# Srecharan/Leaf-Grasping-Vision-ML

Measured on AMD Instinct MI355X. Metric: frames/sec (1080p depth+mask) grasp scoring, 1/8 MI355X; % HBM roofline, higher is better.
Workload: dtype f32; 1 GPU; 1080x1920 depth+mask, 8 score planes + valid + top-20 NMS + GraspPointCNN fp32 rescoring of 20 candidates; height=1080, width=1920, batches_in_flight=1, parallelism=frames sharded over 1 GPU(s), no collective

## Files before the change

### include/leafgrasp.h

```cpp
#ifndef LEAFGRASP_H
#define LEAFGRASP_H

#include <stdint.h>

#ifdef __cplusplus
extern "C" {
#endif

typedef struct lg_ctx* lg_handle;

typedef enum lg_status {
    LG_OK = 0,
    LG_ERR_INVALID = -1,
    LG_ERR_HIP = -2,
    LG_ERR_NOMEM = -3,
    LG_ERR_NO_MODEL = -4,
    LG_ERR_UNSUPPORTED = -5,
    LG_ERR_BUSY = -6
} lg_status;

enum {
    LG_MAP_SDF = 0,
    LG_MAP_APPROACH = 1,
    LG_MAP_FLATNESS = 2,
// ... 161 lines not shown

int lg_debug_dt_max(lg_handle h, int frame, uint32_t out[2], int32_t win[4]);
int lg_debug_dt_form(lg_handle h, int frame, int32_t form[2]);
int lg_debug_dt_search_form(lg_handle h, int32_t* algo);
int lg_dt_form_host(int forced, int n, int H, int W);
int lg_debug_orient_redo(lg_handle h, int32_t* n);
int lg_near_tile_rect(int bx0, int bx1, int by0, int by1, int H, int W, int halo, int32_t rect[4]);
int lg_stem_words_host(const uint64_t* bits, int H, int W, int WW, int bottom_start, int k, uint64_t* out);
int lg_stem_words_host_spans(const uint64_t* bits, int H, int W, int WW, int bottom_start, int n, int anchor, const int8_t* lo,
                             const int8_t* hi, int algo, uint64_t* out);
int lg_stem_plan(int k, int n, int anchor, const int8_t* lo, const int8_t* hi, int32_t* i0, int8_t span_lo[64], int8_t span_hi[64],
                 int8_t dlo[64], int8_t dhi[64]);
int lg_window_from_box(const uint32_t box[5], int H, int W, int search_mode, int32_t out[12]);
int lg_border_line_max(const int32_t* prof, int n, int lo, int len, uint32_t* out);
int lg_debug_near_tiles(lg_handle h, int32_t* off, int cap);
int lg_debug_cnn_scored(lg_handle h, int64_t* patches);
int lg_debug_leaf_fallback(lg_handle h, int32_t* flags, int cap, int32_t* n_frames, int32_t* n_flagged);
int lg_debug_cnn_survivors(lg_handle h, int32_t* sub_frames, int32_t* n_sub, int32_t* counts, int32_t counts_cap,
                           int32_t* list, int32_t* slot, float* logits, int64_t cap, int64_t* n_slots);
int lg_debug_patch(lg_handle h, int64_t slot, float* out);
int lg_debug_isolation_fields(lg_handle h, int frame, uint32_t* dc_fix, uint32_t* dw_fix, uint32_t max_fix[2]);
int lg_label_aware_check(const lg_params* p, int has_labels);
int lg_norm3_host(const int32_t* dx, const int32_t* dy, int n, uint32_t* out);
int lg_dilate_words_host(const uint64_t* bits, int H, int W, int WW, int k, uint64_t* out);
int lg_debug_ws_plane_bytes(lg_handle h, int64_t bytes[LG_NUM_MAPS]);
int lg_wave_rows_on_mask(const uint64_t* bits, int H, int WW, int y, int w);

typedef struct lg_trainer lg_trainer;
typedef struct lg_train_hparams {
    float lr, beta1, beta2, eps, weight_decay;
// ... 40 lines not shown
```

### leaf-grasping-vision-ml_amd/_lib.py

```python
import ctypes as C
import os

_HERE = os.path.dirname(os.path.abspath(__file__))
LIB_PATH = os.environ.get("LG_LIB_PATH") or os.path.join(_HERE, "liblgrasp.so")

LG_NUM_MAPS = 8
MAP_NAMES = ("sdf_score", "approach_score", "flatness_map", "isolation_map", "distance_map",
             "accessibility_map", "stem_penalty", "traditional_score")
MAP_INDEX = {n: i for i, n in enumerate(MAP_NAMES)}

LG_OK, LG_ERR_INVALID, LG_ERR_HIP, LG_ERR_NOMEM, LG_ERR_NO_MODEL, LG_ERR_UNSUPPORTED, LG_ERR_BUSY = 0, -1, -2, -3, -4, -5, -6


class LgParams(C.Structure):
    _fields_ = [(n, C.c_double) for n in ("cx", "cy", "f")] + [(n, C.c_float) for n in (
        "w_approach", "w_sdf", "w_flat", "w_access", "sdf_w_interior", "sdf_w_align",
        "sdf_w_sdf", "optimal_distance", "access_w_dist", "access_w_dir", "flat_scale", "iso_w_close",
        "iso_w_wide", "iso_ramp_top", "iso_ramp_bottom", "min_edge_distance", "stem_valid_thresh")] + \
        [(n, C.c_int32) for n in ("stem_se", "stem_bottom_div", "top_k", "nms_min_distance",
                                  "pregrasp_clearance", "mask_is_bool", "gaussian_size", "chamfer_init_dist0", "label_aware")]


_FP = C.POINTER(C.c_float)

# ... 87 lines not shown
    "lg_debug_dt_max": (C.c_int, [_VP, C.c_int, C.POINTER(C.c_uint32), C.POINTER(C.c_int32)]),
    "lg_format_grasp_results": (C.c_int, [_VP, C.c_int, C.c_char_p, C.c_int64, C.POINTER(C.c_int64)]),
    "lg_debug_dt_form": (C.c_int, [_VP, C.c_int, C.POINTER(C.c_int32)]),
    "lg_debug_orient_redo": (C.c_int, [_VP, C.POINTER(C.c_int32)]),
    "lg_debug_dt_search_form": (C.c_int, [_VP, C.POINTER(C.c_int32)]),
    "lg_dt_form_host": (C.c_int, [C.c_int, C.c_int, C.c_int, C.c_int]),
    "lg_near_tile_rect": (C.c_int, [C.c_int, C.c_int, C.c_int, C.c_int, C.c_int, C.c_int, C.c_int, C.POINTER(C.c_int32)]),
    "lg_stem_words_host": (C.c_int, [_VP, C.c_int, C.c_int, C.c_int, C.c_int, C.c_int, _VP]),
    "lg_stem_words_host_spans": (C.c_int, [_VP, C.c_int, C.c_int, C.c_int, C.c_int, C.c_int, C.c_int, C.POINTER(C.c_int8),
                                           C.POINTER(C.c_int8), C.c_int, _VP]),
    "lg_stem_plan": (C.c_int, [C.c_int, C.c_int, C.c_int, C.POINTER(C.c_int8), C.POINTER(C.c_int8), C.POINTER(C.c_int32),
                               C.POINTER(C.c_int8), C.POINTER(C.c_int8), C.POINTER(C.c_int8), C.POINTER(C.c_int8)]),
    "lg_window_from_box": (C.c_int, [C.POINTER(C.c_uint32), C.c_int, C.c_int, C.c_int, C.POINTER(C.c_int32)]),
    "lg_border_line_max": (C.c_int, [C.POINTER(C.c_int32), C.c_int, C.c_int, C.c_int, C.POINTER(C.c_uint32)]),
    "lg_debug_near_tiles":(C.c_int, [_VP, C.POINTER(C.c_int32), C.c_int]),
    "lg_debug_cnn_scored": (C.c_int, [_VP, C.POINTER(C.c_int64)]),
    "lg_debug_leaf_fallback": (C.c_int, [_VP, C.POINTER(C.c_int32), C.c_int, C.POINTER(C.c_int32), C.POINTER(C.c_int32)]),
    "lg_debug_cnn_survivors": (C.c_int, [_VP, C.POINTER(C.c_int32), C.POINTER(C.c_int32), C.POINTER(C.c_int32), C.c_int32,
                                         C.POINTER(C.c_int32), C.POINTER(C.c_int32), _FP, C.c_int64, C.POINTER(C.c_int64)]),
    "lg_debug_patch": (C.c_int, [_VP, C.c_int64, _FP]),
    "lg_debug_isolation_fields": (C.c_int, [_VP, C.c_int, _VP, _VP, C.POINTER(C.c_uint32)]),
    "lg_label_aware_check": (C.c_int, [C.POINTER(LgParams), C.c_int]),
    "lg_norm3_host": (C.c_int, [_VP, _VP, C.c_int, _VP]),
    "lg_dilate_words_host": (C.c_int, [_VP, C.c_int, C.c_int, C.c_int, C.c_int, _VP]),
    "lg_debug_ws_plane_bytes": (C.c_int, [_VP, C.POINTER(C.c_int64)]),
    "lg_wave_rows_on_mask": (C.c_int, [_VP, C.c_int, C.c_int, C.c_int, C.c_int]),
    "lg_harvest_patches": (C.c_int, [_VP, _VP, _VP, _VP, C.c_int, C.c_int, C.c_int, _VP, _VP, _VP, _VP, _VP, _VP, _VP]),
    "lg_negative_masks": (C.c_int, [_VP, _VP, _VP, C.c_int, C.c_int, _VP, _VP, _VP]),
    "lg_leaf_contour": (C.c_int, [_VP, _VP, C.c_int, C.c_int, _VP, C.c_int, C.POINTER(C.c_int), _VP]),
    "lg_train_create": (C.c_int, [C.c_int, C.c_int, C.POINTER(C.c_int32), C.c_int, C.c_int, C.POINTER(_VP)]),
# ... 55 lines not shown
```

### leaf-grasping-vision-ml_amd/csrc/lg_api.hip

```cpp
#include <math.h>
#include <stdio.h>
#include <stdlib.h>
#include <string.h>

#include <algorithm>
#include <chrono>
#include <functional>
#include <string>
#include <atomic>
#include <memory>
#include <sched.h>
#include <condition_variable>
#include <mutex>
#include <thread>
#include <vector>

#include "lg_cnn.h"
#include "lg_dt.h"
#include "lg_eval.h"
#include "lg_leaf.h"
#include "lg_internal.h"
#include "lg_midrib.h"
#include "lg_orient.h"
#include "lg_pool.h"
// ... 20 lines not shown
    hipEvent_t ev_prep = nullptr, ev_copy = nullptr;
    hipStream_t s_dt[2] = {nullptr, nullptr}, s_main = nullptr, s_topk = nullptr;
    std::vector<hipEvent_t> ev_pool;
    hipEvent_t ev_begin = nullptr;
    int capB = 0, capH = 0, capW = 0, capK = 0;
    uint32_t* tmp = nullptr;
    unsigned long long *bits = nullptr, *stem = nullptr, *tilekeys = nullptr;
    uint8_t* tile_state = nullptr;
    int32_t* near_off = nullptr;
    int32_t* near_off_host = nullptr;
    hipEvent_t ev_near = nullptr;
    int32_t* near_off_host_dev = nullptr;
    LgFrameParams* fp_host_dev = nullptr;
    lg_grasp_result* res_host_dev = nullptr;
    int last_redo = 0;
    int last_near_B = 0;
    uint32_t* maxfix = nullptr;
    uint8_t* mask_ws = nullptr;
    size_t mask_ws_cap = 0;
    unsigned long long *iso_others = nullptr, *iso_dil = nullptr;
    uint32_t* iso_mf = nullptr;
    size_t iso_words_cap = 0;
    int iso_B_cap = 0;
    int last_iso_B = 0, last_iso_H = 0, last_iso_W = 0;
    int32_t* ids_dev = nullptr;
    int32_t* ids_host = nullptr;
    int ids_cap = 0;
    LgWin* win = nullptr;
    LgFrameParams* fp_dev = nullptr;
    LgFrameParams* fp_host = nullptr;
// ... 25 lines not shown
    LgOrientWs* orient = nullptr;
    hipEvent_t ev_orient = nullptr, ev_side = nullptr, ev_search = nullptr;
    int opt_dt_algo = 0;
    int last_dt_algo = 0;
    int opt_dt_band_p = 16, opt_dt_band_e = 4;
    int opt_dt_search = 2;
    int prof_on = 0;
    std::vector<LgProfSlot> prof;
    int host_threads = 8;
    LgPool* pool = nullptr;
    int opt_subbatch = 0;
    bool opt_trace = false;
    int opt_no_skip = 0;
    int opt_final_near = LG_FINAL_NEAR_TPW;
    bool opt_defer_planes = true;
    long long last_patch_floats = 0;
    bool opt_nt_stores = false;
    int opt_side_tail = 1;
    int opt_stem_algo = 1;
    bool opt_direct_host = true;
    bool export_pending = false;
    std::string orient_note;
    std::atomic<bool> busy{false};
    hipStream_t s_cnn = nullptr;
    hipEvent_t ev_cnn0 = nullptr, ev_cnn1 = nullptr;
    bool opt_host_orient = false;
    LgMidribWs* midrib = nullptr;
    void* eval_ws = nullptr;
    size_t eval_cap = 0;
};
// ... 72 lines not shown
        p.used = 0;
    }
}

template <typename T>
hipError_t dev_alloc(T** p, size_t n) {
    return hipMalloc((void**)p, n * sizeof(T));
}

void free_ws(lg_ctx* h) {
    auto F = [](void* p) { if (p) hipFree(p); };
    F(h->tmp); F(h->bits); F(h->stem); F(h->tilekeys); F(h->tile_state); F(h->maxfix); F(h->win); F(h->fp_dev);
    for (int i = 0; i < LG_NUM_MAPS; i++) { F(h->ws_maps_base[i]); h->ws_maps_base[i] = h->ws_maps[i] = nullptr; }
    F(h->ws_valid); F(h->cand_xy); F(h->cand_n); F(h->cand_info); F(h->patches); F(h->logits);
    F(h->surv_keep); F(h->surv_list); F(h->surv_slot); F(h->surv_count);
    F(h->near_off); h->near_off = nullptr; h->last_near_B = 0; h->last_iso_B = 0;
    h->surv_keep = nullptr; h->surv_list = h->surv_slot = h->surv_count = nullptr;
    h->last_scored = 0; h->last_scored_subs = 0; h->last_cnn_B = 0; h->last_patch_floats = 0;
    auto HF = [](void* p) { if (p) hipHostFree(p); };
    HF(h->fp_host); HF(h->bits_host); HF(h->win_host); HF(h->res_host); HF(h->near_off_host);
    h->near_off_host = nullptr;
    h->near_off_host_dev = nullptr; h->fp_host_dev = nullptr; h->res_host_dev = nullptr;
    F(h->res_dev);
    h->tmp = nullptr; h->bits = h->stem = h->tilekeys = nullptr; h->tile_state = nullptr; h->maxfix = nullptr; h->win = nullptr; h->fp_dev = nullptr;
    h->ws_valid = nullptr; h->cand_xy = h->cand_n = nullptr; h->cand_info = h->patches = h->logits = nullptr;
    h->fp_host = nullptr; h->bits_host = nullptr; h->win_host = nullptr; h->bits_host_dev = nullptr; h->res_dev = h->res_host = nullptr;
    h->capB = h->capH = h->capW = h->capK = 0;
}

int ensure_ws(lg_ctx* h, int B, int H, int W, int K) {
    if (B <= h->capB && H == h->capH && W == h->capW && K <= h->capK) return LG_OK;
// ... 141 lines not shown
        return LG_ERR_HIP;
    }
    unsigned hw = std::thread::hardware_concurrency();
    {
        cpu_set_t set;
        CPU_ZERO(&set);
        if (sched_getaffinity(0, sizeof(set), &set) == 0 && CPU_COUNT(&set) > 0) hw = (unsigned)CPU_COUNT(&set);
    }
    unsigned ranks = 1;
    if (const char* e = getenv("LOCAL_WORLD_SIZE")) ranks = (unsigned)std::max(1, atoi(e));
    h->host_threads = (int)std::max(1u, std::min((hw ? hw : 1u) / ranks, 16u));
    if (const char* e = getenv("LG_HOST_THREADS")) h->host_threads = std::max(1, atoi(e));
    if (const char* e = getenv("LG_SUBBATCH")) h->opt_subbatch = std::max(1, atoi(e));
    h->opt_trace = getenv("LG_TRACE") != nullptr;
    if (const char* e = getenv("LG_NO_SKIP")) h->opt_no_skip = std::max(1, atoi(e)) & 3;
    if (const char* e = getenv("LG_FINAL_NEAR")) h->opt_final_near = std::max(0, std::min(64, atoi(e)));
    if (getenv("LG_FINAL_PERSIST") || getenv("LG_FINAL_TPW")) h->opt_final_near = 0;
    h->opt_nt_stores = getenv("LG_NT_STORES") != nullptr;
    h->opt_host_orient = getenv("LG_HOST_ORIENT") != nullptr;
    if (const char* e = getenv("LG_CNN_PRUNE")) h->opt_cnn_prune = atoi(e) != 0;
    if (const char* e = getenv("LG_DEFER_PLANES")) h->opt_defer_planes = atoi(e) != 0;
    if (const char* e = getenv("LG_DT_SEARCH")) h->opt_dt_search = std::max(0, std::min(2, atoi(e)));
    if (const char* e = getenv("LG_DT_SEARCH_ALGO")) {
        const int f = atoi(e);
        if (f == 0 || f == LG_DT_FORM_ROWS || f == LG_DT_FORM_BANDS || f == LG_DT_FORM_SWEEP) h->opt_dt_algo = f;
    }
    if (const char* e = getenv("LG_DT_BAND_P")) { const int p = atoi(e); if (p == 12 || p == 16 || p == 24 || p == 32) h->opt_dt_band_p = p; }
    if (const char* e = getenv("LG_DT_BAND_E")) { const int v = atoi(e); if (v == 2 || v == 4) h->opt_dt_band_e = v; }
    if (const char* e = getenv("LG_SIDE_TAIL")) h->opt_side_tail = std::max(0, std::min(2, atoi(e)));
    if (const char* e = getenv("LG_STEM_ALGO")) h->opt_stem_algo = atoi(e) != 0;
// ... 318 lines not shown
    for (int i = 0; i < n; i++)
        if (prof[i] < -1 || prof[i] > 16384) return LG_ERR_INVALID;
    lg_border_search(prof, n, lo, len, out);
    return LG_OK;
}

int lg_debug_near_tiles(lg_handle h, int32_t* off, int cap) {
    if (!h || !off) return LG_ERR_INVALID;
    LG_ENTER(h);
    if (h->last_near_B <= 0 || !h->near_off_host) return fail(h, LG_ERR_INVALID, "lg_debug_near_tiles: the last call did not take the near launch");
    if (cap < h->last_near_B + 1) return fail(h, LG_ERR_INVALID, "lg_debug_near_tiles: cap must hold B + 1 entries");
    memcpy(off, h->near_off_host, sizeof(int32_t) * (h->last_near_B + 1));
    return LG_OK;
}

int lg_debug_orient_redo(lg_handle h, int32_t* n) {
    if (!h || !n) return LG_ERR_INVALID;
    LG_ENTER(h);
    *n = h->last_redo;
    return LG_OK;
}

int lg_debug_dt_form(lg_handle h, int frame, int32_t form[2]) {
    if (!h || !form || frame < 0 || frame >= h->capB || !h->win) return LG_ERR_INVALID;
    LG_ENTER(h);
    hipSetDevice(h->device);
    hipDeviceSynchronize();
    LgWin w;
    if (hipMemcpy(&w, h->win + frame, sizeof(w), hipMemcpyDeviceToHost) != hipSuccess)
        return fail(h, LG_ERR_HIP, "lg_debug_dt_form: copy failed");
// ... 92 lines not shown
    {
        LgSeSpans se;
        lg_make_se_spans(pl.P.stem_se, &se);
        const int third = pl.H / pl.P.stem_bottom_div;
        LgStemPlan sp;
        lg_make_stem_plan(se, &sp);
        ProfScope ps(h, "stem", s);
        lg_launch_stem_bits(h->bits + off * words, h->stem + off * words, h->win + off, n, pl.H, pl.W, pl.WW,
                            third ? pl.H - third : 0, se, h->opt_stem_algo ? &sp : nullptr, s);
    }
    return LG_OK;
}

int enq_prep(lg_ctx* h, const Plan& pl, int off, int n, hipStream_t s, hipEvent_t ev_prep) {
    h->export_pending = true;
    const size_t px = (size_t)pl.H * pl.W, words = (size_t)pl.H * pl.WW;
    LG_HIP(h, hipMemsetAsync(h->maxfix + LG_MF * (size_t)off, 0, sizeof(uint32_t) * LG_MF * n, s));
    if (pl.label_aware) LG_HIP(h, hipMemsetAsync(h->iso_mf + LG_ISO_MF * (size_t)off, 0, sizeof(uint32_t) * LG_ISO_MF * n, s));
    {
        ProfScope ps(h, "prep", s);
        if (pl.labels && pl.label_aware)
            lg_launch_pack_labels(pl.labels + off * px, h->ids_dev + off, h->mask_ws + off * px, h->bits + off * words, n, pl.H, pl.W,
                                  pl.WW, s, h->maxfix + LG_MF * (size_t)off, h->iso_others + off * words, h->iso_mf + LG_ISO_MF * (size_t)off);
        else if (pl.labels)
            lg_launch_pack_labels(pl.labels + off * px, h->ids_dev + off, h->mask_ws + off * px, h->bits + off * words, n, pl.H, pl.W,
                                  pl.WW, s, h->maxfix + LG_MF * (size_t)off);
        else
            lg_launch_pack_bits(pl.mask + off * px, h->bits + off * words, n, pl.H, pl.W, pl.WW, s, h->maxfix + LG_MF * (size_t)off);
    }
    {
// ... 161 lines not shown
    a.iso_w_close = P.iso_w_close; a.iso_w_wide = P.iso_w_wide;
    a.iso_ramp_top = P.iso_ramp_top; a.iso_ramp_bottom = P.iso_ramp_bottom;
    {
        uint32_t dmax = (uint32_t)((std::min(H, W) + 1) / 2);
        float mx = (float)((uint32_t)P.chamfer_init_dist0 + dmax * LG_A3) * (1.0f / 65536.0f);
        a.init0 = (uint32_t)P.chamfer_init_dist0;
        a.iso_inv_max = 1.0f / mx;
    }
    a.min_edge_distance = P.min_edge_distance; a.stem_valid_thresh = P.stem_valid_thresh;
    a.inv_maxd = (float)(1.0 / sqrt((double)W * W + (double)H * H));
    a.inv_2s2 = 1.0f / (2.0f * P.optimal_distance * P.optimal_distance);
    a.iso_ramp_step = (H > 1) ? (P.iso_ramp_bottom - P.iso_ramp_top) / (float)(H - 1) : 0.0f;
    gaussian1d(P.gaussian_size, a.k1);
    a.gauss_r = P.gaussian_size / 2;
    a.no_skip = h->opt_no_skip;
    a.persist = 0;
    a.nt_stores = h->opt_nt_stores ? 1 : 0;
    if (pl.near) {
        LG_HIP(h, hipEventSynchronize(h->ev_near));
        a.near_off = h->near_off;
        a.near_total = h->near_off_host[n];
        a.near_tpw = h->opt_final_near;
    }
    {
        ProfScope ps(h, "final", s, true);
        lg_launch_final(a, s, ps.slot ? ps.e0 : nullptr, ps.slot ? ps.e1 : nullptr);
    }
    if (keep) *keep = a;
    return LG_OK;
}
// ... 169 lines not shown
    for (int i = 0; i < n && i < cap; i++) { out_xy[2 * i] = pts[2 * i]; out_xy[2 * i + 1] = pts[2 * i + 1]; }
    return LG_OK;
}

int lg_leaf_orientation(lg_handle h, const uint8_t* mask, int H, int W, float* out, int* found, void* stream_) {
    if (!h) return LG_ERR_INVALID;
    LG_ENTER(h);
    if (!mask || !out || !found || H < 1 || W < 1) return fail(h, LG_ERR_INVALID, "lg_leaf_orientation: bad argument");
    hipStream_t s = (hipStream_t)stream_;
    LG_HIP(h, hipSetDevice(h->device));
    int rc = ensure_ws(h, 1, H, W, 20);
    if (rc) return rc;
    const int WW = (W + 63) / 64;
    LG_HIP(h, hipMemsetAsync(h->maxfix, 0, sizeof(uint32_t) * LG_MF, s));
    lg_launch_pack_bits(mask, h->bits, 1, H, W, WW, s, h->maxfix);
    double o[5];
    if (h->orient) {
        lg_launch_window(h->maxfix, h->win, 1, H, W, 0, s);
        lg_launch_orient(h->orient, h->bits, h->win, h->fp_dev, 0, 1, H, W, WW, s);
        LG_HIP(h, hipMemcpyAsync(h->orient->h_out, h->orient->out, sizeof(double) * 5, hipMemcpyDeviceToHost, s));
        LG_HIP(h, hipMemcpyAsync(h->orient->h_status, h->orient->status, sizeof(int), hipMemcpyDeviceToHost, s));
        LG_HIP(h, hipStreamSynchronize(s));
        if (!h->orient->h_status[0]) {
            *found = !std::isnan(h->orient->h_out[0]);
            for (int i = 0; i < 5; i++) out[i] = *found ? (float)h->orient->h_out[i] : NAN;
            return LG_OK;
        }
    }
    LG_HIP(h, hipMemcpyAsync(h->bits_host, h->bits, sizeof(unsigned long long) * (size_t)H * WW, hipMemcpyDeviceToHost, s));
    LG_HIP(h, hipStreamSynchronize(s));
// ... 463 lines not shown
            if (rc) return rc;
            pl.maps[i] = h->ws_maps[i];
        }
    if (!pl.valid) pl.valid = h->ws_valid;
    const int K = P.top_k;
    const size_t px = (size_t)H * W;
    const int tiles = pl.tiles_x * pl.tiles_y;

    int SB = B;
    if (h->opt_subbatch > 0 && !pl.label_aware) SB = h->opt_subbatch;
    const int nsub = (B + SB - 1) / SB;
    const bool piped = nsub > 1;
    std::vector<LgFinalArgs> fargs((size_t)nsub);
    pl.near = pl.sparse && h->opt_final_near > 0 && h->opt_subbatch == 0 && h->opt_no_skip == 0;
    h->last_near_B = 0;
    hipStream_t sD[2] = {piped ? h->s_dt[0] : s, piped ? h->s_dt[1] : s};
    hipStream_t sM = piped ? h->s_main : s, sT = piped ? h->s_topk : s;
    while ((int)h->ev_pool.size() < 6 * nsub) {
        hipEvent_t e;
        LG_HIP(h, hipEventCreateWithFlags(&e, hipEventDisableTiming));
        h->ev_pool.push_back(e);
    }
    auto EV = [&](int k, int which) { return h->ev_pool[6 * k + which]; };
    if (piped) {
        LG_HIP(h, hipEventRecord(h->ev_begin, s));
        for (hipStream_t q : {sD[0], sD[1], sM, sT}) LG_HIP(h, hipStreamWaitEvent(q, h->ev_begin, 0));
    }
    const LgIsoFields iso_fields = {h->tmp, h->iso_mf};
    auto enq_G = [&](int k) -> int {
        const int off = k * SB, n = std::min(SB, B - off);
// ... 129 lines not shown
    }
    if (!h->res_host_dev)
        LG_HIP(h, hipMemcpyAsync(h->res_host, h->res_dev, sizeof(lg_grasp_result) * B, hipMemcpyDeviceToHost, s));
    if (cands)
        LG_HIP(h, hipMemcpyAsync(h->cand_rows_host, h->cand_rows_dev, sizeof(lg_grasp_candidate) * B * K, hipMemcpyDeviceToHost, s));
    const double t_enq2 = now();
    LG_HIP(h, hipStreamSynchronize(s));
    const double t_sync = now();
    LG_HIP(h, hipGetLastError());
    if (use_cnn && lg_cnn_take_error(&h->cnn)) return fail(h, LG_ERR_HIP, "lg_select_grasp: a split CNN item did not receive its parts");
    memcpy(results, h->res_host, sizeof(lg_grasp_result) * B);
    if (cands) memcpy(cands, h->cand_rows_host, sizeof(lg_grasp_candidate) * B * K);
    if (use_cnn) { h->last_cnn_B = B; h->last_cnn_K = K; h->last_cnn_SB = SB; h->last_cnn_pruned = prune; }
    h->last_patch_floats = use_cnn ? (long long)B * K * lg_cnn_halo_patch_floats() : 0;
    if (pl.near) h->last_near_B = B;
    if (pl.label_aware) { h->last_iso_B = B; h->last_iso_H = H; h->last_iso_W = W; }
    if (trace && !piped) {
        float a[5] = {0};
        for (int i = 1; i <= 4; i++) hipEventElapsedTime(&a[i], tev[0], tev[i]);
        fprintf(stderr, "[lg] gpu timeline (ms since call start): sweeps done %.3f | planes %.3f | topk %.3f | cnn %.3f\n", a[1], a[2],
                a[3], a[4]);
    }
    if (trace) for (auto& e : tev) if (e) hipEventDestroy(e);
    if (trace)
        fprintf(stderr, "[lg] B=%d enq1 %.3f | wait bits %.3f | orient %.3f | enq2 %.3f | gpu wait %.3f | post %.3f ms\n", B,
                t_enq1 - t_start, t_copy - t_enq1, t_orient - t_copy, t_enq2 - t_orient, t_sync - t_enq2, now() - t_sync);
    return LG_OK;
}

}
// ... 1 lines not shown
```

### leaf-grasping-vision-ml_amd/csrc/lg_internal.h

```cpp
#pragma once
#include <hip/hip_runtime.h>
#include <stdint.h>

#include "../../include/leafgrasp.h"

#define LG_A5 65536u
#define LG_B5 91750u
#define LG_C5 143976u
#define LG_A3 62587u
#define LG_B3 89738u
#define LG_INIT0 0x1FFFFFFFu
#define LG_INF 0x3FFFFFFFu
#define LG_NOSRC 0x20000000u
#define LG_HCAP 16383u
#ifndef LG_SEARCH_BUDGET
#define LG_SEARCH_BUDGET 2.0e7f
#endif
#define LG_MF 8
#define LG_BOX_X0 2
#define LG_BOX_X1 3
#define LG_BOX_Y0 4
#define LG_BOX_Y1 5
#define LG_BOX_AREA 6

// ... 291 lines not shown
    float access_w_dist, access_w_dir, flat_scale;
    float iso_w_close, iso_w_wide, iso_ramp_top, iso_ramp_bottom, iso_inv_max;
    float min_edge_distance, stem_valid_thresh;
    float inv_maxd;
    uint32_t init0;
    float inv_2s2, iso_ramp_step;
    float k1[7];
    int gauss_r;
    int no_skip;
    int nt_stores;
    int persist;
    int tpw;
    const int32_t* near_off;
    int near_total;
    int near_tpw;
};

void lg_launch_pack_bits(const uint8_t* mask, unsigned long long* bits, int B, int H, int W, int WW, hipStream_t s,
                         uint32_t* mf = nullptr);
void lg_launch_pack_labels(const int16_t* labels, const int32_t* ids_dev, uint8_t* mask, unsigned long long* bits, int B, int H,
                           int W, int WW, hipStream_t s, uint32_t* mf = nullptr, unsigned long long* others = nullptr,
                           uint32_t* iso_mf = nullptr);
void lg_launch_export_rows(const unsigned long long* bits, const LgWin* wins, unsigned long long* dst_host_devptr, int B,
                           int H, int WW, hipStream_t s);
void lg_launch_stem_bits(const unsigned long long* bits, unsigned long long* stem, const LgWin* wins, int B, int H, int W, int WW,
                         int bottom_start, const LgSeSpans& se, const LgStemPlan* plan, hipStream_t s);
void lg_launch_final(const LgFinalArgs& a, hipStream_t s, hipEvent_t ev_start = nullptr, hipEvent_t ev_stop = nullptr);
void lg_launch_near_tiles(const LgWin* win, int B, int H, int W, int halo, int32_t* near_off, int32_t* near_off_host_dev,
                          unsigned long long* tilekeys, uint8_t* tile_state, hipStream_t s);
void lg_launch_smooth(const float* src, float* dst, int B, int H, int W, int S, const LgGaussTaps& taps, hipStream_t s);
// ... 99 lines not shown
```

### leaf-grasping-vision-ml_amd/csrc/lg_kernels.hip

```cpp
#include "lg_internal.h"
#include "lg_wave.h"

#include <hip/hip_ext.h>

#include <limits.h>
#include <algorithm>
#include <type_traits>
#include <stdlib.h>

#define LG_MAX64_STEP(CTRL, RMASK)                                                            \
    {                                                                                         \
        const uint32_t oh = (uint32_t)__builtin_amdgcn_update_dpp(0, (int)hi, CTRL, RMASK, 0xf, false); \
        const uint32_t ol = (uint32_t)__builtin_amdgcn_update_dpp(0, (int)lo, CTRL, RMASK, 0xf, false); \
        const bool take = (oh > hi) || (oh == hi && ol > lo);                                 \
        hi = take ? oh : hi;                                                                  \
        lo = take ? ol : lo;                                                                  \
    }
__device__ __forceinline__ unsigned long long lg_wave_max_u64(unsigned long long v) {
    uint32_t hi = (uint32_t)(v >> 32), lo = (uint32_t)v;
    LG_MAX64_STEP(0x111, 0xf)
    LG_MAX64_STEP(0x112, 0xf)
    LG_MAX64_STEP(0x114, 0xf)
    LG_MAX64_STEP(0x118, 0xf)
    LG_MAX64_STEP(0x142, 0xa)
// ... 89 lines not shown
        if (lane == 0) { fb[wid] = b; if (mf) acc.add(b, w * 64, row, H, W); }
    }
    if (mf) lg_box_flush(acc, s_box, mf + (size_t)frame * LG_MF);
}

__global__ __launch_bounds__(256) void lg_pack_bits16_kernel(const uint8_t* __restrict__ mask,
                                                             unsigned long long* __restrict__ bits, int H, int W, int WW,
                                                             uint32_t* __restrict__ mf) {
    __shared__ uint32_t s_box[5];
    const int slots_per_row = 4 * WW, frame = blockIdx.y;
    const int nslots = H * slots_per_row;
    const uint8_t* fm = mask + (size_t)frame * H * W;
    unsigned long long* fb = bits + (size_t)frame * H * WW;
    LgBoxAcc acc;
    const int stride = gridDim.x * 256;
    for (int sid = blockIdx.x * 256 + threadIdx.x; sid < nslots; sid += stride) {
        const int row = sid / slots_per_row;
        const int slot = sid - row * slots_per_row;
        const int x = slot * 16;
        unsigned b16 = 0;
        if (x < W) {
            const uint4 v = *reinterpret_cast<const uint4*>(fm + (size_t)row * W + x);
            const uint32_t w4[4] = {v.x, v.y, v.z, v.w};
#pragma unroll
            for (int q = 0; q < 4; q++) {
                b16 |= ((w4[q] & 0x000000ffu) ? 1u : 0u) << (4 * q);
                b16 |= ((w4[q] & 0x0000ff00u) ? 2u : 0u) << (4 * q);
                b16 |= ((w4[q] & 0x00ff0000u) ? 4u : 0u) << (4 * q);
                b16 |= ((w4[q] & 0xff000000u) ? 8u : 0u) << (4 * q);
            }
        }
        if (mf) acc.add(b16, x, row, H, W);
        unsigned long long word = (unsigned long long)b16 << (16 * (slot & 3));
        word |= __shfl_xor(word, 1, 64);
        word |= __shfl_xor(word, 2, 64);
        if ((slot & 3) == 0) fb[(size_t)row * WW + (slot >> 2)] = word;
    }
    if (mf) lg_box_flush(acc, s_box, mf + (size_t)frame * LG_MF);
}

static unsigned lg_pack_blocks(long long units, int B, long long target) {
    const long long full = (units + 255) / 256;
    return (unsigned)std::max<long long>(1, std::min<long long>(full, target / B));
}

void lg_launch_pack_bits(const uint8_t* mask, unsigned long long* bits, int B, int H, int W, int WW, hipStream_t s, uint32_t* mf) {
    if ((W & 15) == 0 && ((uintptr_t)mask & 15) == 0) {
        hipLaunchKernelGGL(lg_pack_bits16_kernel, dim3(lg_pack_blocks((long long)H * WW * 4, B, 16384), B), dim3(256), 0, s, mask, bits,
                           H, W, WW, mf);
        return;
    }
// ... 255 lines not shown

template <bool VEC, bool ALL, int R, bool SCORE = false>
__global__ __launch_bounds__(256) LG_FINAL_WPE_ATTR void lg_final_kernel(LgFinalArgs a_) {
    static_assert(!(ALL && SCORE), "score-only stores fewer planes than ALL");
    constexpr int HALO = R + 1;
    static_assert(R >= 0 && HALO <= 4, "the depth tile carries 4 halo columns");
    constexpr int DW = 72;
    constexpr int DH = LG_TH + 2 * HALO;
    constexpr int GW = LG_TW + 2;
    constexpr int GH = LG_TH + 2;
    __shared__ __attribute__((aligned(16))) float s_dm[DH * DW];
    __shared__ float s_h[DH * GW];
    float* const s_g = s_dm;
    static_assert(GH * (GW + 2) <= DH * DW, "g tile must fit in the depth tile");
    __shared__ unsigned long long s_key[4];
    __shared__ int s_any[2];
    typedef float lg_f4 __attribute__((ext_vector_type(4)));
    typedef const __attribute__((address_space(4))) LgFinalArgs* lg_args_ptr;
    lg_args_ptr ap = (lg_args_ptr)__builtin_amdgcn_kernarg_segment_ptr();
    (void)a_;

    const int ntile = ap->tiles_x * ap->tiles_y;
    typedef const __attribute__((address_space(4))) int32_t* lg_off_ptr;
    const bool near = ap->near_off != nullptr;
    const int total = near ? ap->near_total : ntile * ap->B;
    const int xcd = (int)(blockIdx.x & 7u), tq = total >> 3, tr = total & 7;
    const int xcd_first = xcd < tr ? xcd * (tq + 1) : tr * (tq + 1) + (xcd - tr) * tq;
    const int xcd_count = tq + (xcd < tr ? 1 : 0);
    const int tpw = near ? ap->near_tpw : ap->tpw;
    const int stride = tpw > 0 ? 1 : (int)((gridDim.x + 7u) >> 3);
    int it = (int)(blockIdx.x >> 3) * (tpw > 0 ? tpw : 1);
// ... 74 lines not shown
        }
    };
    auto st_valid = [&](unsigned off, int x0, uint32_t vbytes) {
        if (!ALL && !SCORE && !ap->valid) return;
        uint8_t* p = ap->valid + fo + off;
        if (vec) {
            __builtin_nontemporal_store(vbytes, reinterpret_cast<uint32_t*>(p));
        } else {
#pragma unroll
            for (int j = 0; j < 4; j++)
                if (x0 + j < W) p[j] = (uint8_t)((vbytes >> (8 * j)) & 1u);
        }
    };
    float zero = 0.0f;
    asm volatile("" : "+v"(zero));
    if (!ap->no_skip) {
        bool any = false;
        if (near_leaf) {
            if (t < 64) {
                unsigned long long nz = 0;
                for (int e = t; e < DH * 3; e += 64) {
                    const int er = e / 3, wq = e % 3;
                    const int y = lg_reflect(ty0 - HALO + er, H), wi = bx - 1 + wq;
                    if (wi >= 0 && wi < WW) {
                        unsigned long long v = bits_at(bits, y, wi);
                        if (wq == 0) v >>= 56;
                        if (wq == 2) v &= 0xffull;
                        nz |= v;
                    }
                }
                const bool anyw = __ballot(nz != 0) != 0ull;
                if (t == 0) s_any[par] = anyw ? 1 : 0;
            }
            lg_lds_barrier();
            any = s_any[par] != 0;
            par ^= 1;
        }
        if (!any) {
            if (!ap->sparse) {
                const float flat1 = lg_const_flat(ap->flat_scale);
                const float tr1 = ap->w_flat * flat1;
                const float c_flat[4] = {flat1, flat1, flat1, flat1};
                const float c_trad[4] = {tr1, tr1, tr1, tr1};
                const float c_zero[4] = {zero, zero, zero, zero};
#pragma unroll
                for (int rr = 0; rr < RPT; rr++) {
                    const int y = ty0 + tyi + 16 * rr, x0 = tx0 + 4 * txi;
                    if (y < H && x0 < W) {
                        const unsigned off = (unsigned)(y * W + x0);
                        st4(LG_MAP_SDF, off, x0, c_zero); st4(LG_MAP_APPROACH, off, x0, c_zero); st4(LG_MAP_FLATNESS, off, x0, c_flat);
                        st4(LG_MAP_ISOLATION, off, x0, c_zero); st4(LG_MAP_ACCESS, off, x0, c_zero); st4(LG_MAP_STEM, off, x0, c_zero);
                        st4(LG_MAP_TRADITIONAL, off, x0, c_trad);
                        if (!in_win) st4(LG_MAP_DISTANCE, off, x0, c_zero);
                        st_valid(off, x0, 0u);
                    }
                }
            }
            if (t == 0) {
                const int ymax = min(ty0 + LG_TH, H) - 1, xmax = min(tx0 + LG_TW, W) - 1;
                ap->tilekeys[(size_t)frame * ntile + tile] =
                    ((unsigned long long)lg_orderable(0.0f) << 32) | (uint32_t)(ymax * W + xmax);
                if (ap->tile_state) ap->tile_state[(size_t)frame * ntile + tile] = 0;
            }
            continue;
        }
    }

    float din_pre[RPT][4];
    unsigned mnib_pre[RPT], snib_pre[RPT];
#pragma unroll
    for (int rr = 0; rr < RPT; rr++) {
        const int y = ty0 + tyi + 16 * rr, x0 = tx0 + 4 * txi;
        mnib_pre[rr] = snib_pre[rr] = 0;
#pragma unroll
        for (int j = 0; j < 4; j++) din_pre[rr][j] = 0.0f;
        if (y < H && x0 < W) {
            const unsigned sh = (unsigned)(x0 & 63);
            mnib_pre[rr] = (unsigned)(bits_at(bits, y, bx) >> sh) & 0xfu;
            snib_pre[rr] = (unsigned)(bits_at(stemb, y, bx) >> sh) & 0xfu;
            const char* dsrc = (const char*)(ap->maps[LG_MAP_DISTANCE] + fo) + (unsigned)(y * W + x0) * 4u;
            if (!in_win) {
            } else if (vec) {
                float4 v = *reinterpret_cast<const float4*>(dsrc);
                din_pre[rr][0] = v.x; din_pre[rr][1] = v.y; din_pre[rr][2] = v.z; din_pre[rr][3] = v.w;
            } else {
#pragma unroll
                for (int j = 0; j < 4; j++) din_pre[rr][j] = (x0 + j < W) ? reinterpret_cast<const float*>(dsrc)[j] : 0.0f;
            }
        }
    }

    const bool fast = VEC && (tx0 >= 4) && (tx0 + LG_TW + 4 <= W);
    if (fast) {
        for (int idx = t; idx < DH * (DW / 4); idx += 256) {
            int er = idx / (DW / 4), g4 = idx % (DW / 4);
            int y = lg_reflect(ty0 - HALO + er, H);
            int x = tx0 - 4 + 4 * g4;
            float4 d = *reinterpret_cast<const float4*>(depth + (unsigned)(y * W + x) * 4u);
            unsigned long long wbits = bits_at(bits, y, x >> 6);
            unsigned nib = (unsigned)(wbits >> (x & 63)) & 0xfu;
            float4 o;
            o.x = (nib & 1u) ? d.x : 0.0f;
            o.y = (nib & 2u) ? d.y : 0.0f;
            o.z = (nib & 4u) ? d.z : 0.0f;
            o.w = (nib & 8u) ? d.w : 0.0f;
            *reinterpret_cast<float4*>(&s_dm[er * DW + 4 * g4]) = o;
        }
    } else {
// ... 1020 lines not shown
```

### leaf-grasping-vision-ml_amd/grasp_point_selector.py

```python
import ctypes as C
import math
import os
import threading

import numpy as np
import torch

from . import _lib
from ._lib import LG_NUM_MAPS, MAP_NAMES, LgGraspCandidate, LgGraspResult, LgParams, check, lib
from ._log import logerr, loginfo, logwarn
from .cnn import pack_state_dict
from .image_processor import flatness_config

_RESULT_DTYPE = np.dtype([(n, np.int32 if t is C.c_int else np.float32) for n, t in LgGraspResult._fields_])
assert _RESULT_DTYPE.itemsize == C.sizeof(LgGraspResult)
GRASP_CANDIDATE_DTYPE = np.dtype([(n, np.int32 if t is C.c_int32 else np.float32) for n, t in LgGraspCandidate._fields_])
assert GRASP_CANDIDATE_DTYPE.itemsize == C.sizeof(LgGraspCandidate)
_ML_FIELDS = ("ml_score", "ml_confidence", "combined")

_VP = C.c_void_p

MIDRIB_FOUND, MIDRIB_NO_CONTOUR, MIDRIB_THIN, MIDRIB_TOO_FEW = 0, 1, 2, 3


# ... 166 lines not shown
                                             valid.data_ptr(), theta, self._stream()), "lg_score_maps")
        squeeze = (leaf_mask.dim() if hasattr(leaf_mask, "dim") else leaf_mask.ndim) == 2
        out = {n: (maps[i, 0] if squeeze else maps[i]) for i, n in enumerate(MAP_NAMES)}
        th = [None if math.isnan(t) else float(t) for t in theta]
        return out, (valid[0] if squeeze else valid), (th[0] if squeeze else th)

    def dt_maxima(self, frame=0):
        import ctypes as C
        out, win = (C.c_uint32 * 2)(), (C.c_int32 * 4)()
        rc = lib.lg_debug_dt_max(self._h, int(frame), out, win)
        if rc != 0:
            raise RuntimeError(lib.lg_last_error(self._h).decode())
        scale = np.float32(1.0 / 65536.0)
        return np.float32(out[0]) * scale, np.float32(out[1]) * scale, tuple(win)

    def dt_form(self, frame=0):
        import ctypes as C
        form = (C.c_int32 * 2)()
        rc = lib.lg_debug_dt_form(self._h, int(frame), form)
        if rc != 0:
            raise RuntimeError(lib.lg_last_error(self._h).decode())
        return bool(form[0]), bool(form[1])

    def dt_search_form(self):
        import ctypes as C
        algo = C.c_int32()
        rc = lib.lg_debug_dt_search_form(self._h, C.byref(algo))
        if rc != 0:
            raise RuntimeError(lib.lg_last_error(self._h).decode())
        return int(algo.value)
# ... 355 lines not shown
```

Before: 134,300 frames/s.

## Overlap tile skip test with depth prefetch and batch mask bit packing

In the final scoring kernel, near-leaf tiles on the fast path now issue their depth and mask-word loads into registers before the any-mask ballot test. The empty-tile check then spreads across up to four waves, so the skip test and the global loads overlap instead of running back to back. The pack-bits kernel now handles four slots per thread per trip, with a branchless byte-nonzero-to-nibble trick and batched loads to raise memory-level parallelism. Debug accessors for tile state and packed bit rows are added. The cost is that empty tiles now issue loads that are thrown away, and register pressure rises from the prefetch arrays.

```diff
diff --git a/include/leafgrasp.h b/include/leafgrasp.h
--- a/include/leafgrasp.h
+++ b/include/leafgrasp.h
@@ -199,6 +199,8 @@
 int lg_window_from_box(const uint32_t box[5], int H, int W, int search_mode, int32_t out[12]);
 int lg_border_line_max(const int32_t* prof, int n, int lo, int len, uint32_t* out);
 int lg_debug_near_tiles(lg_handle h, int32_t* off, int cap);
+int lg_debug_tile_state(lg_handle h, int frame, uint8_t* out, int cap);
+int lg_debug_bit_rows(lg_handle h, int frame, uint64_t* bits, int64_t cap, uint32_t box[5]);
 int lg_debug_cnn_scored(lg_handle h, int64_t* patches);
 int lg_debug_leaf_fallback(lg_handle h, int32_t* flags, int cap, int32_t* n_frames, int32_t* n_flagged);
 int lg_debug_cnn_survivors(lg_handle h, int32_t* sub_frames, int32_t* n_sub, int32_t* counts, int32_t counts_cap,
diff --git a/leaf-grasping-vision-ml_amd/_lib.py b/leaf-grasping-vision-ml_amd/_lib.py
--- a/leaf-grasping-vision-ml_amd/_lib.py
+++ b/leaf-grasping-vision-ml_amd/_lib.py
@@ -125,6 +125,8 @@
     "lg_window_from_box": (C.c_int, [C.POINTER(C.c_uint32), C.c_int, C.c_int, C.c_int, C.POINTER(C.c_int32)]),
     "lg_border_line_max": (C.c_int, [C.POINTER(C.c_int32), C.c_int, C.c_int, C.c_int, C.POINTER(C.c_uint32)]),
     "lg_debug_near_tiles":(C.c_int, [_VP, C.POINTER(C.c_int32), C.c_int]),
+    "lg_debug_tile_state": (C.c_int, [_VP, C.c_int, C.POINTER(C.c_uint8), C.c_int]),
+    "lg_debug_bit_rows": (C.c_int, [_VP, C.c_int, C.POINTER(C.c_uint64), C.c_int64, C.POINTER(C.c_uint32)]),
     "lg_debug_cnn_scored": (C.c_int, [_VP, C.POINTER(C.c_int64)]),
     "lg_debug_leaf_fallback": (C.c_int, [_VP, C.POINTER(C.c_int32), C.c_int, C.POINTER(C.c_int32), C.POINTER(C.c_int32)]),
     "lg_debug_cnn_survivors": (C.c_int, [_VP, C.POINTER(C.c_int32), C.POINTER(C.c_int32), C.POINTER(C.c_int32), C.c_int32,
diff --git a/leaf-grasping-vision-ml_amd/csrc/lg_api.hip b/leaf-grasping-vision-ml_amd/csrc/lg_api.hip
--- a/leaf-grasping-vision-ml_amd/csrc/lg_api.hip
+++ b/leaf-grasping-vision-ml_amd/csrc/lg_api.hip
@@ -58,6 +58,8 @@
     LgFrameParams* fp_host_dev = nullptr;
     lg_grasp_result* res_host_dev = nullptr;
     int last_redo = 0;
+    int last_state_B = 0, last_state_tiles = 0;
+    int last_bits_B = 0, last_bits_H = 0, last_bits_WW = 0;
     int last_near_B = 0;
     uint32_t* maxfix = nullptr;
     uint8_t* mask_ws = nullptr;
@@ -113,6 +115,7 @@
     int opt_no_skip = 0;
     int opt_final_near = LG_FINAL_NEAR_TPW;
     bool opt_defer_planes = true;
+    int opt_final_trip = 1;
     long long last_patch_floats = 0;
     bool opt_nt_stores = false;
     int opt_side_tail = 1;
@@ -215,7 +218,7 @@
     for (int i = 0; i < LG_NUM_MAPS; i++) { F(h->ws_maps_base[i]); h->ws_maps_base[i] = h->ws_maps[i] = nullptr; }
     F(h->ws_valid); F(h->cand_xy); F(h->cand_n); F(h->cand_info); F(h->patches); F(h->logits);
     F(h->surv_keep); F(h->surv_list); F(h->surv_slot); F(h->surv_count);
-    F(h->near_off); h->near_off = nullptr; h->last_near_B = 0; h->last_iso_B = 0;
+    F(h->near_off); h->near_off = nullptr; h->last_near_B = 0; h->last_state_B = 0; h->last_bits_B = 0; h->last_iso_B = 0;
     h->surv_keep = nullptr; h->surv_list = h->surv_slot = h->surv_count = nullptr;
     h->last_scored = 0; h->last_scored_subs = 0; h->last_cnn_B = 0; h->last_patch_floats = 0;
     auto HF = [](void* p) { if (p) hipHostFree(p); };
@@ -387,6 +390,7 @@
     if (const char* e = getenv("LG_SUBBATCH")) h->opt_subbatch = std::max(1, atoi(e));
     h->opt_trace = getenv("LG_TRACE") != nullptr;
     if (const char* e = getenv("LG_NO_SKIP")) h->opt_no_skip = std::max(1, atoi(e)) & 3;
+    if (const char* e = getenv("LG_FINAL_TRIP")) h->opt_final_trip = atoi(e) != 0 ? 1 : 0;
     if (const char* e = getenv("LG_FINAL_NEAR")) h->opt_final_near = std::max(0, std::min(64, atoi(e)));
     if (getenv("LG_FINAL_PERSIST") || getenv("LG_FINAL_TPW")) h->opt_final_near = 0;
     h->opt_nt_stores = getenv("LG_NT_STORES") != nullptr;
@@ -735,6 +739,32 @@
     return LG_OK;
 }
 
+int lg_debug_tile_state(lg_handle h, int frame, uint8_t* out, int cap) {
+    if (!h || !out) return LG_ERR_INVALID;
+    LG_ENTER(h);
+    if (h->last_state_B <= 0 || !h->tile_state) return fail(h, LG_ERR_INVALID, "lg_debug_tile_state: the last call was not a sparse lg_select_grasp call");
+    if (frame < 0 || frame >= h->last_state_B) return fail(h, LG_ERR_INVALID, "lg_debug_tile_state: no such frame in the last call");
+    if (cap < h->last_state_tiles) return fail(h, LG_ERR_INVALID, "lg_debug_tile_state: cap must hold the frame's tiles");
+    hipSetDevice(h->device);
+    if (hipMemcpy(out, h->tile_state + (size_t)frame * h->last_state_tiles, (size_t)h->last_state_tiles, hipMemcpyDeviceToHost) != hipSuccess)
+        return fail(h, LG_ERR_HIP, "lg_debug_tile_state: copy failed");
+    return LG_OK;
+}
+
+int lg_debug_bit_rows(lg_handle h, int frame, uint64_t* bits, int64_t cap, uint32_t box[5]) {
+    if (!h || !bits || !box) return LG_ERR_INVALID;
+    LG_ENTER(h);
+    const int64_t words = (int64_t)h->last_bits_H * h->last_bits_WW;
+    if (h->last_bits_B <= 0 || !h->bits || !h->maxfix) return fail(h, LG_ERR_INVALID, "lg_debug_bit_rows: no plane call has packed a mask on this workspace");
+    if (frame < 0 || frame >= h->last_bits_B || cap < words) return fail(h, LG_ERR_INVALID, "lg_debug_bit_rows: no such frame, or cap below H * WW");
+    hipSetDevice(h->device);
+    hipDeviceSynchronize();
+    if (hipMemcpy(bits, h->bits + (size_t)frame * words, sizeof(uint64_t) * (size_t)words, hipMemcpyDeviceToHost) != hipSuccess ||
+        hipMemcpy(box, h->maxfix + (size_t)frame * LG_MF + LG_BOX_X0, sizeof(uint32_t) * 5, hipMemcpyDeviceToHost) != hipSuccess)
+        return fail(h, LG_ERR_HIP, "lg_debug_bit_rows: copy failed");
+    return LG_OK;
+}
+
 int lg_debug_orient_redo(lg_handle h, int32_t* n) {
     if (!h || !n) return LG_ERR_INVALID;
     LG_ENTER(h);
@@ -857,6 +887,7 @@
 
 int enq_prep(lg_ctx* h, const Plan& pl, int off, int n, hipStream_t s, hipEvent_t ev_prep) {
     h->export_pending = true;
+    h->last_bits_B = off + n; h->last_bits_H = pl.H; h->last_bits_WW = pl.WW;
     const size_t px = (size_t)pl.H * pl.W, words = (size_t)pl.H * pl.WW;
     LG_HIP(h, hipMemsetAsync(h->maxfix + LG_MF * (size_t)off, 0, sizeof(uint32_t) * LG_MF * n, s));
     if (pl.label_aware) LG_HIP(h, hipMemsetAsync(h->iso_mf + LG_ISO_MF * (size_t)off, 0, sizeof(uint32_t) * LG_ISO_MF * n, s));
@@ -1048,6 +1079,7 @@
     gaussian1d(P.gaussian_size, a.k1);
     a.gauss_r = P.gaussian_size / 2;
     a.no_skip = h->opt_no_skip;
+    a.one_trip = h->opt_final_trip;
     a.persist = 0;
     a.nt_stores = h->opt_nt_stores ? 1 : 0;
     if (pl.near) {
@@ -1247,6 +1279,7 @@
     const int WW = (W + 63) / 64;
     LG_HIP(h, hipMemsetAsync(h->maxfix, 0, sizeof(uint32_t) * LG_MF, s));
     lg_launch_pack_bits(mask, h->bits, 1, H, W, WW, s, h->maxfix);
+    h->last_bits_B = 1; h->last_bits_H = H; h->last_bits_WW = WW;
     double o[5];
     if (h->orient) {
         lg_launch_window(h->maxfix, h->win, 1, H, W, 0, s);
@@ -1740,6 +1773,7 @@
     std::vector<LgFinalArgs> fargs((size_t)nsub);
     pl.near = pl.sparse && h->opt_final_near > 0 && h->opt_subbatch == 0 && h->opt_no_skip == 0;
     h->last_near_B = 0;
+    h->last_state_B = h->last_state_tiles = 0;
     hipStream_t sD[2] = {piped ? h->s_dt[0] : s, piped ? h->s_dt[1] : s};
     hipStream_t sM = piped ? h->s_main : s, sT = piped ? h->s_topk : s;
     while ((int)h->ev_pool.size() < 6 * nsub) {
@@ -1899,6 +1933,7 @@
     if (use_cnn) { h->last_cnn_B = B; h->last_cnn_K = K; h->last_cnn_SB = SB; h->last_cnn_pruned = prune; }
     h->last_patch_floats = use_cnn ? (long long)B * K * lg_cnn_halo_patch_floats() : 0;
     if (pl.near) h->last_near_B = B;
+    if (pl.sparse) { h->last_state_B = B; h->last_state_tiles = pl.tiles_x * pl.tiles_y; }
     if (pl.label_aware) { h->last_iso_B = B; h->last_iso_H = H; h->last_iso_W = W; }
     if (trace && !piped) {
         float a[5] = {0};
diff --git a/leaf-grasping-vision-ml_amd/csrc/lg_internal.h b/leaf-grasping-vision-ml_amd/csrc/lg_internal.h
--- a/leaf-grasping-vision-ml_amd/csrc/lg_internal.h
+++ b/leaf-grasping-vision-ml_amd/csrc/lg_internal.h
@@ -329,6 +329,7 @@
     const int32_t* near_off;
     int near_total;
     int near_tpw;
+    int one_trip;
 };
 
 void lg_launch_pack_bits(const uint8_t* mask, unsigned long long* bits, int B, int H, int W, int WW, hipStream_t s,
diff --git a/leaf-grasping-vision-ml_amd/csrc/lg_kernels.hip b/leaf-grasping-vision-ml_amd/csrc/lg_kernels.hip
--- a/leaf-grasping-vision-ml_amd/csrc/lg_kernels.hip
+++ b/leaf-grasping-vision-ml_amd/csrc/lg_kernels.hip
@@ -127,27 +127,38 @@
     unsigned long long* fb = bits + (size_t)frame * H * WW;
     LgBoxAcc acc;
     const int stride = gridDim.x * 256;
-    for (int sid = blockIdx.x * 256 + threadIdx.x; sid < nslots; sid += stride) {
-        const int row = sid / slots_per_row;
-        const int slot = sid - row * slots_per_row;
-        const int x = slot * 16;
-        unsigned b16 = 0;
-        if (x < W) {
-            const uint4 v = *reinterpret_cast<const uint4*>(fm + (size_t)row * W + x);
-            const uint32_t w4[4] = {v.x, v.y, v.z, v.w};
-#pragma unroll
-            for (int q = 0; q < 4; q++) {
-                b16 |= ((w4[q] & 0x000000ffu) ? 1u : 0u) << (4 * q);
-                b16 |= ((w4[q] & 0x0000ff00u) ? 2u : 0u) << (4 * q);
-                b16 |= ((w4[q] & 0x00ff0000u) ? 4u : 0u) << (4 * q);
-                b16 |= ((w4[q] & 0xff000000u) ? 8u : 0u) << (4 * q);
-            }
-        }
-        if (mf) acc.add(b16, x, row, H, W);
-        unsigned long long word = (unsigned long long)b16 << (16 * (slot & 3));
-        word |= __shfl_xor(word, 1, 64);
-        word |= __shfl_xor(word, 2, 64);
-        if ((slot & 3) == 0) fb[(size_t)row * WW + (slot >> 2)] = word;
+    constexpr int G = 4;
+    const int sid0 = blockIdx.x * 256 + threadIdx.x;
+    const int step_row = stride / slots_per_row, step_slot = stride - step_row * slots_per_row;
+    int nrow = sid0 / slots_per_row, nslot = sid0 - nrow * slots_per_row;
+    auto nib4 = [](uint32_t w) {
+        const uint32_t nzb = (((w & 0x7f7f7f7fu) + 0x7f7f7f7fu) | w) & 0x80808080u;
+        return (((nzb >> 7) * 0x00204081u) >> 21) & 0xfu;
+    };
+    for (int base = sid0 - (int)(threadIdx.x & 63u); base < nslots; base += G * stride) {
+        uint4 v[G];
+        int row[G], slot[G];
+#pragma unroll
+        for (int g = 0; g < G; g++) {
+            const int sid = base + (int)(threadIdx.x & 63u) + g * stride;
+            row[g] = nrow;
+            slot[g] = nslot;
+            nslot += step_slot; nrow += step_row;
+            if (nslot >= slots_per_row) { nslot -= slots_per_row; nrow++; }
+            v[g] = make_uint4(0u, 0u, 0u, 0u);
+            if (sid < nslots && slot[g] * 16 < W) v[g] = *reinterpret_cast<const uint4*>(fm + (size_t)row[g] * W + slot[g] * 16);
+            if (sid >= nslots) row[g] = -1;
+        }
+#pragma unroll
+        for (int g = 0; g < G; g++) {
+            const int x = slot[g] * 16;
+            const unsigned b16 = nib4(v[g].x) | (nib4(v[g].y) << 4) | (nib4(v[g].z) << 8) | (nib4(v[g].w) << 12);
+            if (mf) acc.add(b16, x, row[g], H, W);
+            unsigned long long word = (unsigned long long)b16 << (16 * (slot[g] & 3));
+            word |= __shfl_xor(word, 1, 64);
+            word |= __shfl_xor(word, 2, 64);
+            if (row[g] >= 0 && (slot[g] & 3) == 0) fb[(size_t)row[g] * WW + (slot[g] >> 2)] = word;
+        }
     }
     if (mf) lg_box_flush(acc, s_box, mf + (size_t)frame * LG_MF);
 }
@@ -433,7 +444,7 @@
     float* const s_g = s_dm;
     static_assert(GH * (GW + 2) <= DH * DW, "g tile must fit in the depth tile");
     __shared__ unsigned long long s_key[4];
-    __shared__ int s_any[2];
+    __shared__ int s_any[2][4];
     typedef float lg_f4 __attribute__((ext_vector_type(4)));
     typedef const __attribute__((address_space(4))) LgFinalArgs* lg_args_ptr;
     lg_args_ptr ap = (lg_args_ptr)__builtin_amdgcn_kernarg_segment_ptr();
@@ -538,9 +549,78 @@
     };
     float zero = 0.0f;
     asm volatile("" : "+v"(zero));
+    auto const_tile = [&]() {
+        if (!ap->sparse) {
+            const float flat1 = lg_const_flat(ap->flat_scale);
+            const float tr1 = ap->w_flat * flat1;
+            const float c_flat[4] = {flat1, flat1, flat1, flat1};
+            const float c_trad[4] = {tr1, tr1, tr1, tr1};
+            const float c_zero[4] = {zero, zero, zero, zero};
+#pragma unroll
+            for (int rr = 0; rr < RPT; rr++) {
+                const int y = ty0 + tyi + 16 * rr, x0 = tx0 + 4 * txi;
+                if (y < H && x0 < W) {
+                    const unsigned off = (unsigned)(y * W + x0);
+                    st4(LG_MAP_SDF, off, x0, c_zero); st4(LG_MAP_APPROACH, off, x0, c_zero); st4(LG_MAP_FLATNESS, off, x0, c_flat);
+                    st4(LG_MAP_ISOLATION, off, x0, c_zero); st4(LG_MAP_ACCESS, off, x0, c_zero); st4(LG_MAP_STEM, off, x0, c_zero);
+                    st4(LG_MAP_TRADITIONAL, off, x0, c_trad);
+                    if (!in_win) st4(LG_MAP_DISTANCE, off, x0, c_zero);
+                    st_valid(off, x0, 0u);
+                }
+            }
+        }
+        if (t == 0) {
+            const int ymax = min(ty0 + LG_TH, H) - 1, xmax = min(tx0 + LG_TW, W) - 1;
+            ap->tilekeys[(size_t)frame * ntile + tile] =
+                ((unsigned long long)lg_orderable(0.0f) << 32) | (uint32_t)(ymax * W + xmax);
+            if (ap->tile_state) ap->tile_state[(size_t)frame * ntile + tile] = 0;
+        }
+    };
+    constexpr int TEST_WAVES = (DH * 3 + 63) / 64;
+    static_assert(DH * 3 <= 256 && TEST_WAVES <= 4, "one (row, word) pair per thread");
+    constexpr int NST = (DH * (DW / 4) + 255) / 256;
+    const bool fast = VEC && (tx0 >= 4) && (tx0 + LG_TW + 4 <= W);
+    const bool trip = VEC && SCORE && ap->one_trip && !ap->no_skip && near_leaf && fast;
+    float4 d_pre[NST];
+    unsigned long long w_pre[NST];
     if (!ap->no_skip) {
         bool any = false;
-        if (near_leaf) {
+        if (trip) {
+            unsigned long long testw = 0;
+            if (t < DH * 3) {
+                const int er = t / 3, wq = t - 3 * er;
+                const int y = lg_reflect(ty0 - HALO + er, H), wi = bx - 1 + wq;
+                if (wi >= 0 && wi < WW) {
+                    unsigned long long v = bits_at(bits, y, wi);
+                    if (wq == 0) v >>= 56;
+                    if (wq == 2) v &= 0xffull;
+                    testw = v;
+                }
+            }
+#pragma unroll
+            for (int k = 0; k < NST; k++) {
+                const int idx = t + 256 * k;
+                d_pre[k] = make_float4(0.0f, 0.0f, 0.0f, 0.0f);
+                w_pre[k] = 0;
+                if (idx < DH * (DW / 4)) {
+                    const int er = idx / (DW / 4), g4 = idx % (DW / 4);
+                    const int y = lg_reflect(ty0 - HALO + er, H);
+                    const int x = tx0 - 4 + 4 * g4;
+                    d_pre[k] = *reinterpret_cast<const float4*>(depth + (unsigned)(y * W + x) * 4u);
+                    w_pre[k] = bits_at(bits, y, x >> 6);
+                }
+            }
+            if (t < 64 * TEST_WAVES) {
+                const bool anyw = __ballot(testw != 0) != 0ull;
+                if ((t & 63) == 0) s_any[par][t >> 6] = anyw ? 1 : 0;
+            }
+            lg_lds_barrier();
+            int anyi = 0;
+#pragma unroll
+            for (int w = 0; w < TEST_WAVES; w++) anyi |= s_any[par][w];
+            any = __builtin_amdgcn_readfirstlane(anyi) != 0;
+            par ^= 1;
+        } else if (near_leaf) {
             if (t < 64) {
                 unsigned long long nz = 0;
                 for (int e = t; e < DH * 3; e += 64) {
@@ -554,40 +634,13 @@
                     }
                 }
                 const bool anyw = __ballot(nz != 0) != 0ull;
-                if (t == 0) s_any[par] = anyw ? 1 : 0;
+                if (t == 0) s_any[par][0] = anyw ? 1 : 0;
             }
             lg_lds_barrier();
-            any = s_any[par] != 0;
+            any = s_any[par][0] != 0;
             par ^= 1;
         }
-        if (!any) {
-            if (!ap->sparse) {
-                const float flat1 = lg_const_flat(ap->flat_scale);
-                const float tr1 = ap->w_flat * flat1;
-                const float c_flat[4] = {flat1, flat1, flat1, flat1};
-                const float c_trad[4] = {tr1, tr1, tr1, tr1};
-                const float c_zero[4] = {zero, zero, zero, zero};
-#pragma unroll
-                for (int rr = 0; rr < RPT; rr++) {
-                    const int y = ty0 + tyi + 16 * rr, x0 = tx0 + 4 * txi;
-                    if (y < H && x0 < W) {
-                        const unsigned off = (unsigned)(y * W + x0);
-                        st4(LG_MAP_SDF, off, x0, c_zero); st4(LG_MAP_APPROACH, off, x0, c_zero); st4(LG_MAP_FLATNESS, off, x0, c_flat);
-                        st4(LG_MAP_ISOLATION, off, x0, c_zero); st4(LG_MAP_ACCESS, off, x0, c_zero); st4(LG_MAP_STEM, off, x0, c_zero);
-                        st4(LG_MAP_TRADITIONAL, off, x0, c_trad);
-                        if (!in_win) st4(LG_MAP_DISTANCE, off, x0, c_zero);
-                        st_valid(off, x0, 0u);
-                    }
-                }
-            }
-            if (t == 0) {
-                const int ymax = min(ty0 + LG_TH, H) - 1, xmax = min(tx0 + LG_TW, W) - 1;
-                ap->tilekeys[(size_t)frame * ntile + tile] =
-                    ((unsigned long long)lg_orderable(0.0f) << 32) | (uint32_t)(ymax * W + xmax);
-                if (ap->tile_state) ap->tile_state[(size_t)frame * ntile + tile] = 0;
-            }
-            continue;
-        }
+        if (!any) { const_tile(); continue; }
     }
 
     float din_pre[RPT][4];
@@ -614,8 +667,24 @@
         }
     }
 
-    const bool fast = VEC && (tx0 >= 4) && (tx0 + LG_TW + 4 <= W);
-    if (fast) {
+    if (trip) {
+#pragma unroll
+        for (int k = 0; k < NST; k++) {
+            const int idx = t + 256 * k;
+            if (idx < DH * (DW / 4)) {
+                const int er = idx / (DW / 4), g4 = idx % (DW / 4);
+                const int x = tx0 - 4 + 4 * g4;
+                const float4 d = d_pre[k];
+                unsigned nib = (unsigned)(w_pre[k] >> (x & 63)) & 0xfu;
+                float4 o;
+                o.x = (nib & 1u) ? d.x : 0.0f;
+                o.y = (nib & 2u) ? d.y : 0.0f;
+                o.z = (nib & 4u) ? d.z : 0.0f;
+                o.w = (nib & 8u) ? d.w : 0.0f;
+                *reinterpret_cast<float4*>(&s_dm[er * DW + 4 * g4]) = o;
+            }
+        }
+    } else if (fast) {
         for (int idx = t; idx < DH * (DW / 4); idx += 256) {
             int er = idx / (DW / 4), g4 = idx % (DW / 4);
             int y = lg_reflect(ty0 - HALO + er, H);
diff --git a/leaf-grasping-vision-ml_amd/grasp_point_selector.py b/leaf-grasping-vision-ml_amd/grasp_point_selector.py
--- a/leaf-grasping-vision-ml_amd/grasp_point_selector.py
+++ b/leaf-grasping-vision-ml_amd/grasp_point_selector.py
@@ -204,6 +204,24 @@
         scale = np.float32(1.0 / 65536.0)
         return np.float32(out[0]) * scale, np.float32(out[1]) * scale, tuple(win)
 
+    def tile_state(self, frame, H, W):
+        import ctypes as C
+        ty, tx = (int(H) + 15) // 16, (int(W) + 63) // 64
+        out = np.empty(ty * tx, np.uint8)
+        rc = lib.lg_debug_tile_state(self._h, int(frame), out.ctypes.data_as(C.POINTER(C.c_uint8)), out.size)
+        if rc != 0:
+            raise RuntimeError(lib.lg_last_error(self._h).decode())
+        return out.reshape(ty, tx)
+
+    def bit_rows(self, frame, H, W):
+        import ctypes as C
+        bits, box = np.zeros((int(H), (int(W) + 63) // 64), np.uint64), np.zeros(5, np.uint32)
+        rc = lib.lg_debug_bit_rows(self._h, int(frame), bits.ctypes.data_as(C.POINTER(C.c_uint64)), bits.size,
+                                   box.ctypes.data_as(C.POINTER(C.c_uint32)))
+        if rc != 0:
+            raise RuntimeError(lib.lg_last_error(self._h).decode())
+        return bits, box
+
     def dt_form(self, frame=0):
         import ctypes as C
         form = (C.c_int32 * 2)()
```

Measured after the change: 135,400 frames/s, median of 4. Within noise of the previous version (+0.8%).
